# FeMTTU/femus

Hardware: AMD Instinct MI355X
Metric: assembled DOFs/sec + V-cycle SpMV GB/s (% HBM peak), 3D Poisson Q2 (higher is better)
Workload: dtype f64

## Files before the change

### femus_amd/csrc/fh_assemble.hip

```cpp
#include "fh_internal.h"
#include "fh_fe.h"
#include "fh_expr_device.h"
#include <algorithm>

struct SfTab { double L[3][4], D[3][4]; };

struct fh_assembler_s {
  fh_ctx_t ctx = nullptr;
  int geom = 0, fe = 0, order = 0, dim = 3, nc = 27, ng = 64, nloc = 27;
  int nel = 0, nnode = 0, ndof = 0;
  int ncolors = 0;
  std::vector<int> color_ptr;
  int* d_color_elems = nullptr;
  int* d_elem_dof = nullptr;
  double* d_coords = nullptr;
  double* d_w = nullptr;
  double* d_phi = nullptr;
  double* d_dphi = nullptr;
  int* d_emap = nullptr;
  int* d_iota = nullptr;
  int ncp = 28;
  int* d_adj_ptr = nullptr;
  int* d_adj_ei = nullptr;
  unsigned char* d_rowmap = nullptr;
// ... 9 lines not shown
  double *d_gal_val = nullptr, *d_gal_res = nullptr, *d_gal_dense = nullptr;
  int kstride = 27;
  double* d_Fbuf = nullptr;
  bool two_pass = false;
  bool fused = false;
  bool kbuf_valid = false;
  bool rows_used_since = false;
  int last_path = 0;
  int cl_ncl = 0, cl_nm = 0, cl_ns = 0, cl_nprow = 0;
  int cl_sup_shift = 0;
  int cl_walk_shift = 0;
  size_t cl_ncarried = 0;
  size_t cl_npart = 0;
  unsigned* d_cl_sinfo = nullptr;
  void *d_cl_dtab = nullptr, *d_cl_fblk = nullptr, *d_cl_oblk = nullptr;
  int *d_cl_vdst = nullptr, *d_cl_fdst = nullptr;
  unsigned long long* d_cl_vdst64 = nullptr;
  double* cl_val_base = nullptr;
  unsigned char *d_cl_map = nullptr, *d_cl_pmap = nullptr;
  unsigned char* d_cl_mapb = nullptr;
  unsigned short* d_cl_gtab = nullptr;
  bool cl_all_rows = false;
  bool macro_valid = false;
  fh_mat_t cl_mat_of_macro = nullptr;
  uint64_t macro_val_gen = 0;
  double* d_Pbuf = nullptr;
  int* d_cl_prow = nullptr;
  unsigned* d_cl_pstart = nullptr;
  int last_source_kind = 0;
  double last_params[2] = {1.0, 0.0};
// ... 1584 lines not shown
constexpr int CL_LV = CL_ZC + 2;
constexpr size_t CL_OFF_DT = (size_t)(CL_LV + CL_NBLK) * sizeof(double);
constexpr size_t CL_OFF_RB = CL_OFF_DT + (size_t)CL_NS_MAX * 8;
constexpr size_t CL_OFF_FB = CL_OFF_RB + (size_t)CL_NM_MAX * 8;
constexpr size_t CL_OFF_FL = CL_OFF_FB + (size_t)CL_NM_MAX * 4;
constexpr size_t CL_OFF_OV = CL_OFF_FL + (size_t)CL_NM_MAX * 16;
constexpr size_t cl_lds_bytes() { return CL_OFF_OV + (size_t)CL_NBLK * 16; }
static_assert((CL_LV + CL_NBLK) * 8 < (1 << 17), "cluster kernel: LDS byte addresses of the stagings and the long-sum cells fit 17 bits");
static_assert(CL_ZC < (1 << 16), "cluster kernel: 16-bit double indices of the address blocks");
static_assert(cl_lds_bytes() <= 160 * 1024, "cluster kernel: LDS budget");
static_assert((CL_TAB % 2) == 0 && (CL_UVS % 2) == 0, "cluster kernel: 16-byte alignment of the wave regions");

struct ClParams {
  int ncl, ns, nm;
  int sup_shift;
  const uint2* dtab;
  const uint4* fblk;
  const uint4* oblk;
  const unsigned* sinfo;
  const unsigned long long* vdst;
  const int* fdst;
  const uint4* map;
  const uint4* mapb;
  double* Pbuf;
  double* res;
  unsigned long long* stamps;
};

__device__ __forceinline__ double cl_sum8(const char* S, const uint4 a, double t) {
  const unsigned w[4] = {a.x, a.y, a.z, a.w};
// ... 225 lines not shown
        cl_gdouble* dst = (cl_gdouble*)vb[i];
        if (P.debug & 64) *dst = vv[i];
        else if (!(P.debug & 4)) __builtin_nontemporal_store(vv[i], dst);
        else if (vv[i] == 1.2345e300) *dst = vv[i];
      }
      if (CARRY && lane < 16) {
        cl_gdouble* dst = (cl_gdouble*)(fvv < 0 ? C.Pbuf + (size_t)(fvv & 0x7fffffff) : C.res + (size_t)(fvv & 0x3fffffff));
        *dst = (fvv >= 0 && (fvv & 0x40000000)) ? fold + fsum : fsum;
      }
      sf_stamp<INS>(st, 15);
    }
    sf_stamp<INS>(st, 10);
    __syncthreads();
    sf_stamp<INS>(st, 11);
    dof_n = dof_nn;
    ndone++;
  }
  if (INS && C.stamps && lane == 0) {
    unsigned long long* o = C.stamps + ((size_t)blockIdx.x * NW + wave) * 20;
#pragma unroll
    for (int k = 0; k < 16; k++) o[k] = st.acc[k];
    o[16] = (unsigned long long)ndone;
  }
}

constexpr int RP_Q = 7;
template <int NT>
__global__ __launch_bounds__(256) void k_rows_partial(int nprow, const int* __restrict__ prow, const unsigned* __restrict__ pstart, const unsigned char* __restrict__ pmap,
                                                      const double* __restrict__ Pbuf, const int* __restrict__ rowptr, double* __restrict__ val, double* __restrict__ res, int nt) {
  __shared__ double acc[8][2][128];
// ... 290 lines not shown
    FH_CHECK_HIP(hipMemcpyAsync(&perr, d_perr, sizeof(int), hipMemcpyDeviceToHost, ctx->stream));
    FH_CHECK_HIP(hipStreamSynchronize(ctx->stream));
    if (perr) return 0;
  }
  FH_TRACE("cluster plan: clusters verified");
  std::vector<unsigned short> roff(CL_NM_MAX + 1, 0);
  std::vector<unsigned char> tcol;
  int nsingle[CL_NM_MAX] = {};
  struct U2 { unsigned x, y; };
  struct U4 { unsigned short a[8]; };
  std::vector<U2> dtab;
  U4 zblk;
  for (int q = 0; q < 8; q++) zblk.a[q] = (unsigned short)CL_ZC;
  std::vector<U4> fblk(CL_NM_MAX, zblk), oblk;
  auto stag = [&](int e, int tr, int tc) { return (unsigned)(CL_TAB + e * SF_WAVE + SF_XT + tr * KS + tc); };
  auto pack = [&](const std::vector<unsigned>& ad, U2* out) -> bool {
    if (ad.empty() || ad.size() > 8) return false;
    out->x = ad[0] * 8;
    out->y = (ad.size() > 1 ? ad[1] : (unsigned)CL_ZC) * 8;
    if (ad.size() > 2) {
      if ((int)oblk.size() >= CL_NBLK) return false;
      U4 b = zblk;
      for (size_t q = 0; q < ad.size(); q++) b.a[q] = (unsigned short)ad[q];
      out->x = (unsigned)(CL_LV + (int)oblk.size()) * 8;
      out->y = (unsigned)CL_ZC * 8;
      oblk.push_back(b);
    }
    return true;
  };
  int tof_e[CL_NE][CL_NM_MAX];
  for (int e = 0; e < CL_NE; e++) {
    for (int k = 0; k < nm; k++) tof_e[e][k] = -1;
    for (int t = 0; t < 27; t++) tof_e[e][tm[e][t]] = t;
  }
  for (int r = 0; r < nm; r++) {
    bool has[CL_NM_MAX] = {};
    for (int e = 0; e < CL_NE; e++)
      if (tof_e[e][r] >= 0)
        for (int t = 0; t < 27; t++) has[tm[e][t]] = true;
    for (int pass = 0; pass < 2; pass++) {
      for (int k = 0; k < nm; k++)
        if (has[k]) {
          std::vector<unsigned> ad;
          for (int e = 0; e < CL_NE; e++)
            if (tof_e[e][r] >= 0 && tof_e[e][k] >= 0) ad.push_back(stag(e, tof_e[e][r], tof_e[e][k]));
          if ((ad.size() > 1) != (pass == 1)) continue;
          U2 d;
          if (!pack(ad, &d)) return 0;
          dtab.push_back(d);
          tcol.push_back((unsigned char)k);
        }
      if (pass == 0) nsingle[r] = (int)dtab.size() - roff[r];
    }
    roff[r + 1] = (unsigned short)dtab.size();
    if (roff[r + 1] - roff[r] > 127) return 0;
    int nf = 0;
    for (int e = 0; e < CL_NE; e++)
      if (tof_e[e][r] >= 0) fblk[r].a[nf++] = (unsigned short)stag(e, tof_e[e][r], 27);
  }
  for (int r = nm; r < CL_NM_MAX; r++) roff[r + 1] = roff[nm];
  const int ns = (int)dtab.size();
  if (ns > CL_NS_MAX || ns >= (1 << 13)) return 0;
  oblk.resize(CL_NBLK, zblk);
  std::vector<unsigned> sinfo((size_t)CL_SPT * CL_T, (unsigned)(CL_NM_MAX - 1));
  {
    int sidx = 0;
    for (int pass = 0; pass < 2; pass++)
      for (int r = 0; r < nm; r++) {
        const int p0 = pass ? nsingle[r] : 0, p1 = pass ? roff[r + 1] - roff[r] : nsingle[r];
        for (int pp = p0; pp < p1; pp++) sinfo[sidx++] = (unsigned)r | ((unsigned)pp << 7) | ((unsigned)roff[r] << 14);
      }
  }
  FH_TRACE("cluster plan: template");
  for (int r = 0; r <= CL_NM_MAX; r++) T.roff[r] = roff[r];
  unsigned char* d_complete = nullptr;
  unsigned *d_rowsz = nullptr, *d_rowbase = nullptr;
  FH_TRY(dalloc((void**)&d_complete, (size_t)m));
  FH_TRY(dalloc((void**)&d_rowsz, (size_t)m * sizeof(unsigned)));
// ... 41 lines not shown
  FH_CHECK_HIP(hipMalloc(&as->d_cl_vdst, (size_t)ncl * CL_NM_MAX * sizeof(int)));
  FH_CHECK_HIP(hipMalloc(&as->d_cl_fdst, (size_t)ncl * CL_NM_MAX * sizeof(int)));
  hipLaunchKernelGGL(k_cl_dst, dim3(gq), dim3(256), 0, ctx->stream, ncl, m, d_cdof, as->d_adj_ptr, as->d_adj_ei, A->d_rowptr, T, d_complete, d_rowbase, sink,
                     as->d_cl_vdst, as->d_cl_fdst);
  FH_CHECK_HIP(hipGetLastError());
  FH_CHECK_HIP(hipStreamSynchronize(ctx->stream));
  FH_TRACE("cluster plan: destinations");
  auto up = [&](void** d, const void* h, size_t bytes) -> int {
    FH_CHECK_HIP(hipMalloc(d, bytes ? bytes : 8));
    if (bytes) FH_CHECK_HIP(hipMemcpy(*d, h, bytes, hipMemcpyHostToDevice));
    return 0;
  };
  FH_TRY(up((void**)&as->d_cl_dtab, dtab.data(), dtab.size() * sizeof(U2)));
  FH_TRY(up((void**)&as->d_cl_fblk, fblk.data(), fblk.size() * sizeof(U4)));
  FH_TRY(up((void**)&as->d_cl_oblk, oblk.data(), oblk.size() * sizeof(U4)));
  {
    std::vector<unsigned short> gtab((size_t)CL_NE * 27 * 27, (unsigned short)0xffff);
    for (int e = 0; e < CL_NE; e++)
      for (int il = 0; il < 27; il++)
        for (int ic = 0; ic < 27; ic++) {
          const int r = tm[e][T.tof[il]], k = tm[e][T.tof[ic]];
          int owner = -1;
          for (int e2 = 0; e2 < CL_NE && owner < 0; e2++)
            if (tof_e[e2][r] >= 0 && tof_e[e2][k] >= 0) owner = e2;
          if (owner != e) continue;
          for (int idx = roff[r]; idx < roff[r + 1]; idx++)
            if (tcol[idx] == k) gtab[((size_t)e * 27 + il) * 27 + ic] = (unsigned short)idx;
        }
    FH_TRY(up((void**)&as->d_cl_gtab, gtab.data(), gtab.size() * sizeof(unsigned short)));
    as->cl_all_rows = (m == as->nnode);
// ... 25 lines not shown
    FH_CHECK_HIP(hipMemsetAsync(d_ncar, 0, sizeof(unsigned long long), ctx->stream));
    hipLaunchKernelGGL(k_cluster_maps, dim3(ncl), dim3(256), 0, ctx->stream, ncl, ns, nm, d_cdof, as->d_cl_sinfo, d_roff, d_tcol, as->d_cl_vdst, m, A->d_rowptr, A->d_col, d_complete,
                       as->d_adj_ptr, as->d_adj_ei, as->d_elem_dof, nloc, reinterpret_cast<uint4*>(as->d_cl_map), reinterpret_cast<uint4*>(as->d_cl_mapb), as->d_cl_pmap, d_first, d_err);
    if (sup_shift > 0 && m > 0)
      hipLaunchKernelGGL(k_cl_cover, dim3(fh_div_up(m, 256)), dim3(256), 0, ctx->stream, m, A->d_rowptr, d_complete, d_first, d_err, d_ncar);
    FH_CHECK_HIP(hipGetLastError());
    int err = 0;
    unsigned long long ncar = 0;
    FH_CHECK_HIP(hipMemcpyAsync(&err, d_err, sizeof(int), hipMemcpyDeviceToHost, ctx->stream));
    FH_CHECK_HIP(hipMemcpyAsync(&ncar, d_ncar, sizeof(ncar), hipMemcpyDeviceToHost, ctx->stream));
    FH_CHECK_HIP(hipStreamSynchronize(ctx->stream));
    as->cl_ncarried = (size_t)ncar;
    for (void* q : {(void*)d_tcol, (void*)d_roff, (void*)d_err}) hipFree(q);
    if (err && sup_shift > 0) {
      FH_TRACE("fh_assembler_create: carried rows do not cover their CSR rows -- cluster plan without them");
      for (void** q : {(void**)&as->d_cl_dtab, (void**)&as->d_cl_fblk, (void**)&as->d_cl_sinfo, (void**)&as->d_cl_oblk, (void**)&as->d_cl_gtab, (void**)&as->d_cl_vdst, (void**)&as->d_cl_vdst64,
                       (void**)&as->d_cl_fdst, (void**)&as->d_cl_map, (void**)&as->d_cl_mapb, (void**)&as->d_cl_pmap, (void**)&as->d_Pbuf, (void**)&as->d_cl_prow, (void**)&as->d_cl_pstart}) {
        if (*q) FH_CHECK_HIP(hipFree(*q));
        *q = nullptr;
      }
      return cluster_plan_build(as, A, elem_dof, aptr, false);
    }
    if (err) {
      FH_TRACE("fh_assembler_create: cluster maps could not be placed in the matrix pattern -- two-pass assembly kept");
      return 0;
    }
  }
  as->cl_ncl = ncl;
  as->cl_nm = nm;
  as->cl_ns = ns;
  as->cl_npart = npart;
  as->cl_nprow = (int)prow.size();
  as->cl_sup_shift = sup_shift;
  if (sup_shift > 0 || ctx->assemble_carry < 100) as->cl_walk_shift = sup_shift;
  as->fused = true;
  FH_TRACE("fh_assembler_create: cluster plan (%d clusters, %d macro nodes, %d entries; super-clusters of %d: %zu carried entries; %zu partial entries, %d rows in the second pass)", ncl,
           nm, ns, 1 << sup_shift, as->cl_ncarried, npart, as->cl_nprow);
  return 0;
}

template <bool CARRY>
static int launch_cluster_stamped(fh_assembler_t as, const AsmParams& P, const ClParams& C0, int grid) {
  constexpr size_t lds = cl_lds_bytes();
  static bool attr_set[64] = {};
  const int dev = as->ctx->device & 63;
  if (!attr_set[dev]) {
    FH_CHECK_HIP(hipFuncSetAttribute(reinterpret_cast<const void*>(&k_cluster_q2hex_sf<0, true, true, CARRY>), hipFuncAttributeMaxDynamicSharedMemorySize, (int)lds));
    attr_set[dev] = true;
  }
  ClParams C = C0;
  const size_t nst = (size_t)grid * CL_NE * 20;
  FH_CHECK_HIP(hipMalloc(&C.stamps, nst * sizeof(unsigned long long)));
  FH_CHECK_HIP(hipMemsetAsync(C.stamps, 0, nst * sizeof(unsigned long long), as->ctx->stream));
  hipLaunchKernelGGL((k_cluster_q2hex_sf<0, true, true, CARRY>), dim3(grid), dim3(CL_T), lds, as->ctx->stream, P, as->sf_tab, as->d_sfLc, as->d_sfLi, C);
  FH_CHECK_HIP(hipGetLastError());
  std::vector<unsigned long long> h(nst);
  FH_CHECK_HIP(hipMemcpyAsync(h.data(), C.stamps, nst * sizeof(unsigned long long), hipMemcpyDeviceToHost, as->ctx->stream));
  FH_CHECK_HIP(hipStreamSynchronize(as->ctx->stream));
  FH_CHECK_HIP(hipFree(C.stamps));
  static const int order[16] = {0, 1, 2, 3, 4, 5, 6, 7, 8, 9, 12, 14, 13, 15, 10, 11};
  static const char* name[16] = {"loop top (previous barrier exit -> stamp)", "phase A: U (gather x, first contraction, sync)", "phase A: V (second contraction, sync)",
                                 "phase A: J, cofactors, division, D_q", "stage 1 (15 MFMA, writes, sync)", "source 2nd contraction + stages 2-3 (4 x 16 reads + 66 FMA)",
                                 "source 3rd contraction, sync", "destination loads issued, staging writes (18), sync", "residual K_e u, next nodes, destinations",
                                 "workgroup barrier 1 (waiting for the slowest wave)", "(end of the output phase)", "workgroup barrier 2",
                                 "output: descriptors + destinations read, residual entries and long sums", "output: both operands read, added", "output: barrier behind the long sums", "output: stores issued"};
  for (int half = 0; half < 2; half++) {
    double sum[16] = {0}, ncl = 0, tot = 0;
    for (size_t w = 0; w < (size_t)grid * CL_NE; w++) {
      if ((int)((w % CL_NE) / (CL_NE / 2)) != half) continue;
      for (int k = 0; k < 16; k++) sum[k] += (double)h[w * 20 + k];
      ncl += (double)h[w * 20 + 16];
    }
    for (int k = 0; k < 16; k++) tot += sum[k];
    fprintf(stderr, "k_cluster_q2hex_sf<0> phase stamps, waves %d..%d (%s): %d workgroups, %.0f wave-clusters, %.0f shader-clock ticks per cluster and wave\n", half * 4, half * 4 + 3,
            half && !(P.debug & 256) ? "phase A one cluster ahead, i.e. rows 1-3 run behind row 8" : "phase A in place", grid, ncl, tot / std::max(ncl, 1.0));
    for (int kk = 0; kk < 16; kk++) {
      const int k = order[kk];
      fprintf(stderr, "  %2d %-62s %9.1f  %5.1f %%\n", k, name[k], sum[k] / std::max(ncl, 1.0), 100.0 * sum[k] / std::max(tot, 1.0));
    }
  }
  return 0;
}

template <int SRC, bool CARRY>
static int launch_cluster_one(fh_assembler_t as, const AsmParams& P, const ClParams& C) {
  constexpr size_t lds = cl_lds_bytes();
  static bool attr_set[64] = {};
  const int dev = as->ctx->device & 63;
  if (!attr_set[dev]) {
    FH_CHECK_HIP(hipFuncSetAttribute(reinterpret_cast<const void*>(&k_cluster_q2hex_sf<SRC, false, true, CARRY>), hipFuncAttributeMaxDynamicSharedMemorySize, (int)lds));
    attr_set[dev] = true;
  }
  const int grid = std::max(1, std::min(C.ncl >> (CARRY ? C.sup_shift : 0), as->ctx->num_cu * as->ctx->assemble_sf_grid));
  if (SRC == 0 && (as->ctx->asm_debug & 128)) return launch_cluster_stamped<CARRY>(as, P, C, grid);
  hipLaunchKernelGGL((k_cluster_q2hex_sf<SRC, false, true, CARRY>), dim3(grid), dim3(CL_T), lds, as->ctx->stream, P, as->sf_tab, as->d_sfLc, as->d_sfLi, C);
  FH_CHECK_HIP(hipGetLastError());
  return 0;
}

__global__ void k_cluster_vdst(size_t n, const int* __restrict__ vdst, double* Pbuf, double* val, unsigned long long* __restrict__ out) {
  const size_t k = (size_t)blockIdx.x * blockDim.x + threadIdx.x;
  if (k >= n) return;
  const int v = vdst[k];
  out[k] = reinterpret_cast<unsigned long long>(v < 0 ? Pbuf + (size_t)(v & 0x7fffffff) : val + (size_t)v);
}

static int launch_cluster(fh_assembler_t as, const AsmParams& P, fh_mat_t A, double* res) {
  if (as->cl_val_base != A->d_val) {
    const size_t n = (size_t)as->cl_ncl * CL_NM_MAX;
    hipLaunchKernelGGL(k_cluster_vdst, dim3((unsigned)((n + 255) / 256)), dim3(256), 0, as->ctx->stream, n, as->d_cl_vdst, as->d_Pbuf, A->d_val, as->d_cl_vdst64);
    FH_CHECK_HIP(hipGetLastError());
    as->cl_val_base = A->d_val;
  }
  ClParams C;
  C.ncl = as->cl_ncl; C.ns = as->cl_ns; C.nm = as->cl_nm;
  C.dtab = reinterpret_cast<const uint2*>(as->d_cl_dtab); C.fblk = reinterpret_cast<const uint4*>(as->d_cl_fblk); C.oblk = reinterpret_cast<const uint4*>(as->d_cl_oblk);
  C.sinfo = as->d_cl_sinfo;
  C.vdst = as->d_cl_vdst64; C.fdst = as->d_cl_fdst; C.map = reinterpret_cast<const uint4*>(as->d_cl_map); C.mapb = reinterpret_cast<const uint4*>(as->d_cl_mapb);
  C.Pbuf = as->d_Pbuf; C.res = res;
  C.stamps = nullptr;
  C.sup_shift = as->cl_walk_shift;
  if (as->cl_sup_shift > 0 || (as->ctx->assemble_carry >= 200 && as->d_cl_mapb)) {
    if (P.source_kind == 4) FH_TRY((launch_cluster_one<2, true>(as, P, C)));
    else if (P.source_kind != 0) FH_TRY((launch_cluster_one<1, true>(as, P, C)));
    else FH_TRY((launch_cluster_one<0, true>(as, P, C)));
  } else if (P.source_kind == 4) FH_TRY((launch_cluster_one<2, false>(as, P, C)));
  else if (P.source_kind != 0) FH_TRY((launch_cluster_one<1, false>(as, P, C)));
  else FH_TRY((launch_cluster_one<0, false>(as, P, C)));
  if (as->cl_nprow > 0 && !(as->ctx->asm_debug & (2 | 8))) {
    if (!(as->ctx->asm_debug & 32))
      hipLaunchKernelGGL(k_rows_partial<0>, dim3(fh_div_up(as->cl_nprow, 16)), dim3(256), 0, as->ctx->stream, as->cl_nprow, as->d_cl_prow, as->d_cl_pstart,
                         as->d_cl_pmap, as->d_Pbuf, A->d_rowptr, A->d_val, res, 0);
    else
      hipLaunchKernelGGL(k_rows_partial<1>, dim3(fh_div_up(as->cl_nprow, 16)), dim3(256), 0, as->ctx->stream, as->cl_nprow, as->d_cl_prow, as->d_cl_pstart,
                         as->d_cl_pmap, as->d_Pbuf, A->d_rowptr, A->d_val, res, 1);
    FH_CHECK_HIP(hipGetLastError());
  }
  return 0;
}

template <int SRC>
__global__ __launch_bounds__(256) void k_elem_q2hex_affine(AsmParams P, const double* __restrict__ Mab, const double* __restrict__ mphi) {
  constexpr int NC = 27, DIM = 3, EB = 16, NE = NC * NC;
// ... 614 lines not shown
extern "C" int fh_assembler_destroy(fh_assembler_t as) {
  if (!as) return 0;
  hipStreamSynchronize(as->ctx->stream);
  if (as->d_color_elems) hipFree(as->d_color_elems);
  hipFree(as->d_elem_dof);
  hipFree(as->d_coords);
  hipFree(as->d_w);
  hipFree(as->d_phi);
  hipFree(as->d_dphi);
  if (as->d_emap) hipFree(as->d_emap);
  for (void* q : {(void*)as->d_aff_elems, (void*)as->d_gen_elems, (void*)as->d_Mab, (void*)as->d_mphi, (void*)as->d_mfT, (void*)as->d_mfPhi, (void*)as->d_mfSFc, (void*)as->d_mfSFi, (void*)as->d_sfLc, (void*)as->d_sfLi})
    if (q) hipFree(q);
  if (as->d_prog) hipFree(as->d_prog);
  if (as->d_prog_consts) hipFree(as->d_prog_consts);
  hipFree(as->d_iota);
  for (void* q : {(void*)as->d_cl_dtab, (void*)as->d_cl_fblk, (void*)as->d_cl_sinfo, (void*)as->d_cl_oblk, (void*)as->d_cl_gtab, (void*)as->d_cl_vdst, (void*)as->d_cl_vdst64, (void*)as->d_cl_fdst, (void*)as->d_cl_map, (void*)as->d_cl_mapb, (void*)as->d_cl_pmap,
                  (void*)as->d_Pbuf, (void*)as->d_cl_prow, (void*)as->d_cl_pstart})
    if (q) hipFree(q);
  for (void* q : {(void*)as->d_adj_ptr, (void*)as->d_adj_ei, (void*)as->d_rowmap, (void*)as->d_Kbuf, (void*)as->d_Fbuf, (void*)as->d_slot, (void*)as->d_gal_child,
                  (void*)as->d_gal_cnt, (void*)as->d_gal_row, (void*)as->d_gal_fb, (void*)as->d_gal_cb, (void*)as->d_gal_val, (void*)as->d_gal_res, (void*)as->d_gal_dense,
                  (void*)as->d_gal_fmask})
    if (q) hipFree(q);
  delete as;
  return 0;
}

static int assemble_poisson_core(fh_assembler_t as, fh_vec_t sol, int source_kind, const double* params, fh_mat_t A, fh_vec_t res);

extern "C" int fh_assemble_poisson(fh_assembler_t as, fh_vec_t sol, int source_kind, const double* params, fh_mat_t A, fh_vec_t res) {
  FH_REQUIRE(source_kind >= 0 && source_kind <= 3, "fh_assemble_poisson: unknown source kind %d", source_kind);
// ... 1657 lines not shown
```

### femus_amd/csrc/fh_core.hip

```cpp
#include <cstdlib>
#include "fh_internal.h"
#include <chrono>
#include <cstdlib>
#include <cstdarg>
#include <cmath>

static thread_local char g_err[1024] = "";

void fh_set_error(const char* fmt, ...) {
  va_list ap;
  va_start(ap, fmt);
  vsnprintf(g_err, sizeof(g_err), fmt, ap);
  va_end(ap);
}

extern "C" const char* fh_last_error(void) { return g_err; }

bool fh_trace_on() {
  static const bool on = [] {
    const char* e = getenv("FEMUS_HIP_TRACE");
    return e && *e && *e != '0';
  }();
  return on;
}
// ... 181 lines not shown
  else if (!strcmp(name, "spmv_kernel")) c->spmv_kernel = (int)value;
  else if (!strcmp(name, "spmv_nt")) c->spmv_nt = (int)value;
  else if (!strcmp(name, "spmv_share")) c->spmv_share = (int)value;
  else if (!strcmp(name, "spmv_threads")) c->spmv_threads = (int)value;
  else if (!strcmp(name, "assemble_emap")) c->assemble_emap = (int)value;
  else if (!strcmp(name, "asm_debug")) c->asm_debug = (int)value;
  else if (!strcmp(name, "debug_poison")) c->debug_poison = (int)value;
  else if (!strcmp(name, "assemble_two_pass")) c->assemble_two_pass = (int)value;
  else if (!strcmp(name, "assemble_sym")) c->assemble_sym = (int)value;
  else if (!strcmp(name, "assemble_mfma")) c->assemble_mfma = (int)value;
  else if (!strcmp(name, "assemble_kpad")) c->assemble_kpad = (int)value;
  else if (!strcmp(name, "assemble_rows2")) c->assemble_rows2 = (int)value;
  else if (!strcmp(name, "assemble_sf")) c->assemble_sf = (int)value;
  else if (!strcmp(name, "assemble_rows_nt")) c->assemble_rows_nt = (int)value;
  else if (!strcmp(name, "assemble_fused")) c->assemble_fused = (int)value;
  else if (!strcmp(name, "assemble_sf_grid")) c->assemble_sf_grid = std::max(1, (int)value);
  else if (!strcmp(name, "assemble_sumfac")) c->assemble_sumfac = (int)value;
  else if (!strcmp(name, "galerkin_mfma")) c->galerkin_mfma = (int)value;
  else if (!strcmp(name, "gj_block")) c->gj_block = (int)value;
  else if (!strcmp(name, "vanka_persistent")) c->vanka_persistent = (int)value;
  else if (!strcmp(name, "coarse_reduce")) c->coarse_reduce = (int)value;
  else if (!strcmp(name, "coarse_nd")) c->coarse_nd = (int)value;
  else if (!strcmp(name, "coarse_nd_min")) c->coarse_nd_min = (int)value;
  else if (!strcmp(name, "coarse_direct")) c->coarse_direct = (int)value;
  else if (!strcmp(name, "gmres_device")) c->gmres_device = (int)value;
  else if (!strcmp(name, "galerkin_macro")) c->galerkin_macro = (int)value;
  else if (!strcmp(name, "vanka_fused")) c->vanka_fused = (int)value;
  else if (!strcmp(name, "coarse_direct_min")) c->coarse_direct_min = (int)value;
  else if (!strcmp(name, "coarse_nd_streams")) c->coarse_nd_streams = (int)value;
  else if (!strcmp(name, "patch_invert_lds")) c->patch_invert_lds = (int)value;
// ... 344 lines not shown
```

### femus_amd/csrc/fh_internal.h

```cpp
#pragma once
#include <hip/hip_runtime.h>
#include <cstdint>
#include <cstdio>
#include <cstdlib>
#include <cstring>
#include <new>
#include <stdexcept>
#include <string>
#include <algorithm>
#include <vector>
#include "../../include/femus_hip.h"

void fh_set_error(const char* fmt, ...);

#define FH_CHECK_HIP(expr)                                                                        \
  do {                                                                                            \
    hipError_t _e = (expr);                                                                       \
    if (_e != hipSuccess) {                                                                       \
      fh_set_error("%s:%d: %s failed: %s", __FILE__, __LINE__, #expr, hipGetErrorString(_e));     \
      return 1;                                                                                   \
    }                                                                                             \
  } while (0)

#define FH_REQUIRE(cond, ...)                                                                     \
// ... 50 lines not shown
  int spmv_share = 1;
  int spmv_nt = 0;
  int assemble_emap = 1;
  int asm_debug = 0;
  int debug_poison = 0;
  int assemble_mfma = 12;
  int assemble_rows_nt = 1;
  int assemble_sf_grid = 1;
  int assemble_sf = 8;
  int assemble_sumfac = 1;
  int assemble_rows2 = 1;
  int assemble_kpad = 1;
  int assemble_sym = 1;
  int assemble_two_pass = 1;
  int assemble_fused = 1;
  int ilu_ahead = 2;
  int tri_runs = 1;
  int assemble_carry = -1;
  int assemble_affine = 0;
  int gj_symmetric = 1;
  int galerkin_mfma = 1;
  int patch_invert_lds = 1;
  int coarse_nd = 8;
  int coarse_nd_streams = 0;
  int coarse_nd_min = 1024;
  int vanka_fused = 1;
  int galerkin_macro = 1;
  int gmres_device = 1;
  int coarse_direct = 1;
  int coarse_direct_min = 8192;
// ... 124 lines not shown
```

Baseline: 817.7 million.

## Add software-pipelined cluster assembly kernel with packed symmetric staging

```diff
diff --git a/femus_amd/csrc/fh_assemble.hip b/femus_amd/csrc/fh_assemble.hip
--- a/femus_amd/csrc/fh_assemble.hip
+++ b/femus_amd/csrc/fh_assemble.hip
@@ -47,6 +47,7 @@
   size_t cl_npart = 0;
   unsigned* d_cl_sinfo = nullptr;
   void *d_cl_dtab = nullptr, *d_cl_fblk = nullptr, *d_cl_oblk = nullptr;
+  void *d_cl_dtabp = nullptr, *d_cl_fblkp = nullptr, *d_cl_oblkp = nullptr;
   int *d_cl_vdst = nullptr, *d_cl_fdst = nullptr;
   unsigned long long* d_cl_vdst64 = nullptr;
   double* cl_val_base = nullptr;
@@ -1661,6 +1662,7 @@
 struct ClParams {
   int ncl, ns, nm;
   int sup_shift;
+  const unsigned* dtabp;
   const uint2* dtab;
   const uint4* fblk;
   const uint4* oblk;
@@ -1916,6 +1918,298 @@
     __syncthreads();
     sf_stamp<INS>(st, 11);
     dof_n = dof_nn;
+    ndone++;
+  }
+  if (INS && C.stamps && lane == 0) {
+    unsigned long long* o = C.stamps + ((size_t)blockIdx.x * NW + wave) * 20;
+#pragma unroll
+    for (int k = 0; k < 16; k++) o[k] = st.acc[k];
+    o[16] = (unsigned long long)ndone;
+  }
+}
+
+constexpr int CP_NT = 27 * 28 / 2;
+constexpr int CP_ES = CP_NT + 28;
+constexpr int CP_ST = 0;
+constexpr int CP_ZC = CP_ST + CL_NE * CP_ES;
+constexpr int CP_LV = CP_ZC + 2;
+constexpr int CP_TAB = CP_LV + CL_NBLK;
+constexpr int CP_W = CP_TAB + CL_TAB;
+constexpr size_t CP_OFF_DT = (size_t)(CP_W + CL_NE * SF_WAVE) * sizeof(double);
+constexpr size_t CP_OFF_RB = CP_OFF_DT + (size_t)CL_NS_MAX * 4;
+constexpr size_t CP_OFF_FB = CP_OFF_RB + (size_t)CL_NM_MAX * 8;
+constexpr size_t CP_OFF_FL = CP_OFF_FB + (size_t)CL_NM_MAX * 4;
+constexpr size_t CP_OFF_OV = CP_OFF_FL + (size_t)CL_NM_MAX * 16;
+constexpr size_t CP_OFF_SI = CP_OFF_OV + (size_t)CL_NBLK * 16;
+constexpr size_t cp_lds_bytes() { return CP_OFF_SI + (size_t)CL_SPT * CL_T * 4; }
+static_assert((CP_LV + CL_NBLK) * 8 <= 0xffff, "pipelined cluster kernel: 16-bit byte addresses of the stagings, the zero cell and the long-sum cells");
+static_assert(cp_lds_bytes() <= 160 * 1024, "pipelined cluster kernel: LDS budget");
+static_assert((CP_ES % 2) == 0 && (CP_TAB % 2) == 0 && (CP_W % 2) == 0, "pipelined cluster kernel: 16-byte alignment of the regions");
+__host__ __device__ constexpr int cp_packed(int r, int c) { return r >= c ? r * (r + 1) / 2 + c : c * (c + 1) / 2 + r; }
+
+template <int SRC, bool INS = false, bool CARRY = false>
+__global__ __launch_bounds__(CL_T) void k_cluster_q2hex_pipe(AsmParams P, SfTab tab, const double* __restrict__ lanec, const int* __restrict__ lanei, ClParams C) {
+  constexpr int NC = 27, DIM = 3, KS = MF_KS, NW = CL_NE;
+  constexpr bool REGC = true;
+  extern __shared__ __attribute__((aligned(16))) double sf_smem[];
+  double* SFl = sf_smem + CP_TAB;
+  int* SFi = reinterpret_cast<int*>(SFl + (SF_NLC - CL_LC0) * 64);
+  char* Sb = reinterpret_cast<char*>(sf_smem);
+  unsigned* dtab = reinterpret_cast<unsigned*>(Sb + CP_OFF_DT);
+  unsigned long long* rb = reinterpret_cast<unsigned long long*>(Sb + CP_OFF_RB);
+  int* fb = reinterpret_cast<int*>(Sb + CP_OFF_FB);
+  uint4* fblk = reinterpret_cast<uint4*>(Sb + CP_OFF_FL);
+  uint4* oblk = reinterpret_cast<uint4*>(Sb + CP_OFF_OV);
+  unsigned* sitab = reinterpret_cast<unsigned*>(Sb + CP_OFF_SI);
+  const int tid = threadIdx.x;
+  for (int k = tid; k < CL_SPT * CL_T; k += CL_T) sitab[k] = C.sinfo[k];
+  for (int k = tid; k < (SF_NLC - CL_LC0) * 64; k += CL_T) SFl[k] = lanec[CL_LC0 * 64 + k];
+  for (int k = tid; k < SF_NLI * 64; k += CL_T) SFi[k] = lanei[k];
+  for (int k = tid; k < C.ns; k += CL_T) dtab[k] = C.dtabp[k];
+  if (tid < CL_NM_MAX) fblk[tid] = C.fblk[tid];
+  if (tid < CL_NBLK) oblk[tid] = C.oblk[tid];
+  if (tid < 2) sf_smem[CP_ZC + tid] = 0.0;
+  __syncthreads();
+  const int lane = tid & 63;
+  const int wave = __builtin_amdgcn_readfirstlane(tid >> 6);
+  double* xt = sf_smem + CP_W + wave * SF_WAVE;
+  double* R = xt + SF_XT;
+  double* Ks = sf_smem + CP_ST + wave * CP_ES;
+  const double* LCl = SFl + lane - CL_LC0 * 64;
+  const int* LIl = SFi + lane;
+  double rcA[19], rcZ[8], rcY[16];
+#pragma unroll
+  for (int r = 0; r < 19; r++) rcA[r] = lanec[r * 64 + lane];
+#pragma unroll
+  for (int r = 0; r < 8; r++) rcZ[r] = lanec[(19 + r) * 64 + lane];
+#pragma unroll
+  for (int r = 0; r < 16; r++) rcY[r] = lanec[(27 + r) * 64 + lane];
+  unsigned pk0 = (unsigned)lanei[5 * 64 + lane] | ((unsigned)lanei[6 * 64 + lane] << 8) | ((unsigned)lanei[15 * 64 + lane] << 16) | ((unsigned)lanei[14 * 64 + lane] << 24) |
+                 ((lanei[9 * 64 + lane] != 0 ? 1u : 0u) << 29);
+  unsigned pk1;
+  {
+    const int based = lanei[7 * 64 + lane];
+    pk1 = (unsigned)(based / KS) | ((unsigned)(based % KS) << 8);
+  }
+  unsigned pk2 = (unsigned)lanei[lane] | ((unsigned)lanei[64 + lane] << 6) | ((unsigned)lanei[2 * 64 + lane] << 12) | ((unsigned)lanei[3 * 64 + lane] << 18) |
+                 ((unsigned)lanei[4 * 64 + lane] << 24);
+  const int nodeofl = (int)((pk0 >> 24) & 31u);
+  const int cstride = gridDim.x;
+  const int sh = CARRY ? C.sup_shift : 0;
+  const int nsup = C.ncl >> sh;
+  if ((int)blockIdx.x >= nsup) return;
+  const int nit = ((nsup - 1 - (int)blockIdx.x) / cstride + 1) << sh;
+  auto cl_at = [&](int it) {
+    it = min(it, nit - 1);
+    return ((((int)blockIdx.x + (it >> sh) * cstride)) << sh) + (it & ((1 << sh) - 1));
+  };
+  SfStamps st;
+  if (INS) {
+#pragma unroll
+    for (int k = 0; k < 16; k++) st.acc[k] = 0;
+    st.prev = __builtin_amdgcn_s_memtime();
+  }
+  auto element = [&](double (&Kb)[3][3], double& fsrc) {
+    CL_OPAQUE(pk0);
+    CL_OPAQUE(pk2);
+    const int esym = (int)(pk0 & 255u), ens = (int)((pk0 >> 8) & 255u), ensT = (int)((pk0 >> 16) & 255u);
+    const int eout = (lane >> 4) * SF_ES + (lane & 15);
+    double Dr[7];
+    sf_phase_a<SRC, REGC, INS>(P, LCl, CL_IDXA(), rcA, xt, R, Dr, &st);
+    wave_lds_sync();
+    sf_stages<SRC, REGC, INS>(P, tab, LCl, LIl, rcZ, rcY, esym, ens, ensT, eout, R, lane, Dr, Kb, fsrc, &st);
+    sf_stamp<INS>(st, 6);
+  };
+  auto stage_out = [&](const double (&Kb)[3][3], const double fsrc) {
+    CL_OPAQUE(pk0);
+    CL_OPAQUE(pk1);
+    const bool diag = ((pk0 >> 29) & 1u) != 0;
+    const int p = (int)(pk1 & 255u), p2 = (int)(pk1 >> 8);
+    const int bl = (p * (p + 1) >> 1) + p2, bu = (p2 * (p2 + 1) >> 1) + p;
+#pragma unroll
+    for (int a = 0; a < 3; a++)
+#pragma unroll
+      for (int a2 = 0; a2 < 3; a2++) {
+        const double v = (a2 < a && diag) ? Kb[a2][a] : Kb[a][a2];
+        const int idx = a > a2 ? bl + 9 * a * p + (9 * a) * (9 * a + 1) / 2 + 9 * a2 : bu + 9 * a2 * p2 + (9 * a2) * (9 * a2 + 1) / 2 + 9 * a;
+        Ks[idx] = v;
+      }
+    wave_lds_sync();
+    sf_stamp<INS>(st, 7);
+    const int t = min(lane & 31, NC - 1);
+    double ku = 0.0;
+    if (P.sol) {
+      const int h = lane >> 5;
+      const double* ur = xt + 84 + h * 14;
+      const int tt = (t * (t + 1)) >> 1;
+#pragma unroll
+      for (int g = 0; g < 14; g++) {
+        const bool live = g < 13 || h == 0;
+        const int c = h * 14 + g;
+        const int idx = c <= t ? tt + c : ((c * (c + 1)) >> 1) + t;
+        const double v = live ? Ks[idx] : 0.0, uu = live ? ur[g] : 0.0;
+        ku += v * uu;
+      }
+      ku += __shfl_xor(ku, 32, 64);
+    }
+    Ks[CP_NT + t] = -(ku + fsrc);
+  };
+  auto dst_load = [&](int c, unsigned long long& vd, int& fd) {
+    const int tm = tid & (CL_NM_MAX - 1);
+    vd = C.vdst[(size_t)c * CL_NM_MAX + tm];
+    fd = C.fdst[(size_t)c * CL_NM_MAX + tm];
+  };
+  int dof_n;
+  {
+    const int dof = P.elem_dof[(size_t)(cl_at(0) * NW + wave) * P.nloc + nodeofl];
+    if (lane < NC) {
+      xt[lane] = P.coords[(size_t)dof * DIM];
+      xt[28 + lane] = P.coords[(size_t)dof * DIM + 1];
+      xt[56 + lane] = P.coords[(size_t)dof * DIM + 2];
+      xt[84 + lane] = P.sol ? P.sol[dof] : 0.0;
+    }
+    dof_n = P.elem_dof[(size_t)(cl_at(1) * NW + wave) * P.nloc + nodeofl];
+  }
+  wave_lds_sync();
+  double Kb[3][3], fsrc;
+  {
+    unsigned long long vd;
+    int fd;
+    dst_load(cl_at(0), vd, fd);
+    const double nx0 = P.coords[(size_t)dof_n * DIM], nx1 = P.coords[(size_t)dof_n * DIM + 1], nx2 = P.coords[(size_t)dof_n * DIM + 2];
+    const double nu = P.sol ? P.sol[dof_n] : 0.0;
+    const int dof_nn = P.elem_dof[(size_t)(cl_at(2) * NW + wave) * P.nloc + nodeofl];
+    element(Kb, fsrc);
+    stage_out(Kb, fsrc);
+    if (lane < NC) {
+      xt[lane] = nx0;
+      xt[28 + lane] = nx1;
+      xt[56 + lane] = nx2;
+      xt[84 + lane] = nu;
+    }
+    if (tid < CL_NM_MAX) {
+      rb[tid] = vd;
+      fb[tid] = fd;
+    }
+    dof_n = dof_nn;
+  }
+  __syncthreads();
+  int ndone = 0;
+  typedef __attribute__((address_space(1))) double cl_gdouble;
+#pragma unroll 1
+  for (int it = 0; it < nit; it++) {
+    const int cl = cl_at(it);
+    const bool more = it + 1 < nit;
+    const uint4 mp_cur = C.map[(size_t)cl * CL_T + tid];
+    const uint4 mq_cur = CARRY ? C.mapb[(size_t)cl * CL_T + tid] : make_uint4(0u, 0u, 0u, 0u);
+    const int fv_own = CARRY ? C.fdst[(size_t)cl * CL_NM_MAX + wave * 16 + (lane & 15)] : 0;
+    sf_stamp<INS>(st, 0);
+    double nx0 = 0.0, nx1 = 0.0, nx2 = 0.0, nu = 0.0;
+    int dof_nn = 0;
+    if (more) {
+      nx0 = P.coords[(size_t)dof_n * DIM];
+      nx1 = P.coords[(size_t)dof_n * DIM + 1];
+      nx2 = P.coords[(size_t)dof_n * DIM + 2];
+      nu = P.sol ? P.sol[dof_n] : 0.0;
+      dof_nn = P.elem_dof[(size_t)(cl_at(it + 3) * NW + wave) * P.nloc + nodeofl];
+      element(Kb, fsrc);
+      if (lane < NC) {
+        xt[lane] = nx0;
+        xt[28 + lane] = nx1;
+        xt[56 + lane] = nx2;
+      }
+    }
+    unsigned long long vd_nx = 0;
+    int fd_nx = 0;
+    if (more) dst_load(cl_at(it + 1), vd_nx, fd_nx);
+    if (!(P.debug & 2)) {
+      const int frow = wave * 16 + (lane & 15);
+      const uint4 sumblk = (lane & 16) ? oblk[frow] : fblk[frow];
+      const unsigned mw[4] = {mp_cur.x, mp_cur.y, mp_cur.z, mp_cur.w};
+      const unsigned mq[4] = {mq_cur.x, mq_cur.y, mq_cur.z, mq_cur.w};
+      double fold = 0.0;
+      if (CARRY && lane < 16 && fv_own >= 0 && (fv_own & 0x40000000))
+        fold = __hip_atomic_load((const cl_gdouble*)(C.res + (size_t)(fv_own & 0x3fffffff)), __ATOMIC_RELAXED, __HIP_MEMORY_SCOPE_AGENT);
+      unsigned dd[CL_SPT];
+      unsigned long long vb[CL_SPT];
+      double accv[CARRY ? CL_SPT : 1];
+#pragma unroll
+      for (int i = 0; i < CL_SPT; i++) {
+        const unsigned si = sitab[i * CL_T + tid];
+        const int j = (mw[i >> 2] >> (8 * (i & 3))) & 255;
+        const int p = (si >> 7) & 127;
+        const int pos = CARRY ? (int)((mq[i >> 2] >> (8 * (i & 3))) & 255) : p;
+        dd[i] = dtab[(si >> 14) + j];
+        vb[i] = rb[si & 127] + (unsigned long long)(pos * 8);
+      }
+      if (CARRY) {
+#pragma unroll
+        for (int i = 0; i < CL_SPT; i++) {
+          accv[i] = 0.0;
+          if (((mw[2] >> (16 + i)) & 1u) && !(P.debug & 512)) accv[i] = __hip_atomic_load((const cl_gdouble*)vb[i], __ATOMIC_RELAXED, __HIP_MEMORY_SCOPE_AGENT);
+        }
+      }
+      double fsum;
+      int fvv;
+      {
+        const double v = cl_sum8(Sb, sumblk, 0.0);
+        const int fv = CARRY ? fv_own : fb[frow];
+        double* dst = fv < 0 ? C.Pbuf + (size_t)(fv & 0x7fffffff) : C.res + (size_t)(CARRY ? (fv & 0x3fffffff) : fv);
+        if (!CARRY) { if (lane < 16) *dst = v; }
+        if (lane >= 16 && lane < 32) sf_smem[CP_LV + frow] = v;
+        fsum = v;
+        fvv = fv;
+      }
+      if (INS) {
+        asm volatile("" ::"v"(dd[CL_SPT - 1]), "v"(vb[CL_SPT - 1]));
+        sf_stamp<INS>(st, 12);
+      }
+      __syncthreads();
+      sf_stamp<INS>(st, 14);
+      double vv[CL_SPT], ww[CL_SPT];
+#pragma unroll
+      for (int i = 0; i < CL_SPT; i++) {
+        vv[i] = *reinterpret_cast<const double*>(Sb + (dd[i] & 0xffffu));
+        ww[i] = *reinterpret_cast<const double*>(Sb + (dd[i] >> 16));
+      }
+#pragma unroll
+      for (int i = 0; i < CL_SPT; i++) vv[i] += ww[i];
+      if (CARRY) {
+#pragma unroll
+        for (int i = 0; i < CL_SPT; i++) vv[i] = accv[i] + vv[i];
+      }
+      if (INS) {
+        asm volatile("" ::"v"(vv[CL_SPT - 1]), "v"(vv[0]));
+        sf_stamp<INS>(st, 13);
+      }
+#pragma unroll
+      for (int i = 0; i < CL_SPT; i++) {
+        cl_gdouble* dst = (cl_gdouble*)vb[i];
+        if (P.debug & 64) *dst = vv[i];
+        else if (!(P.debug & 4)) __builtin_nontemporal_store(vv[i], dst);
+        else if (vv[i] == 1.2345e300) *dst = vv[i];
+      }
+      if (CARRY && lane < 16) {
+        cl_gdouble* dst = (cl_gdouble*)(fvv < 0 ? C.Pbuf + (size_t)(fvv & 0x7fffffff) : C.res + (size_t)(fvv & 0x3fffffff));
+        *dst = (fvv >= 0 && (fvv & 0x40000000)) ? fold + fsum : fsum;
+      }
+      sf_stamp<INS>(st, 15);
+    }
+    sf_stamp<INS>(st, 10);
+    __syncthreads();
+    sf_stamp<INS>(st, 9);
+    if (more) {
+      stage_out(Kb, fsrc);
+      if (lane < NC) xt[84 + lane] = nu;
+      if (tid < CL_NM_MAX) {
+        rb[tid] = vd_nx;
+        fb[tid] = fd_nx;
+      }
+      dof_n = dof_nn;
+    }
+    sf_stamp<INS>(st, 8);
+    __syncthreads();
+    sf_stamp<INS>(st, 11);
     ndone++;
   }
   if (INS && C.stamps && lane == 0) {
@@ -2236,6 +2530,20 @@
   for (int q = 0; q < 8; q++) zblk.a[q] = (unsigned short)CL_ZC;
   std::vector<U4> fblk(CL_NM_MAX, zblk), oblk;
   auto stag = [&](int e, int tr, int tc) { return (unsigned)(CL_TAB + e * SF_WAVE + SF_XT + tr * KS + tc); };
+  std::vector<unsigned> dtabp;
+  U4 zblkp;
+  for (int q = 0; q < 8; q++) zblkp.a[q] = (unsigned short)CP_ZC;
+  std::vector<U4> fblkp(CL_NM_MAX, zblkp), oblkp;
+  auto stagp = [&](int e, int tr, int tc) { return (unsigned)(CP_ST + e * CP_ES + (tc == 27 ? CP_NT + tr : cp_packed(tr, tc))); };
+  auto packp = [&](const std::vector<unsigned>& ad, unsigned* out) {
+    *out = (ad[0] * 8) | ((ad.size() > 1 ? ad[1] : (unsigned)CP_ZC) * 8) << 16;
+    if (ad.size() > 2) {
+      U4 b = zblkp;
+      for (size_t q = 0; q < ad.size(); q++) b.a[q] = (unsigned short)ad[q];
+      *out = ((unsigned)(CP_LV + (int)oblkp.size()) * 8) | ((unsigned)CP_ZC * 8) << 16;
+      oblkp.push_back(b);
+    }
+  };
   auto pack = [&](const std::vector<unsigned>& ad, U2* out) -> bool {
     if (ad.empty() || ad.size() > 8) return false;
     out->x = ad[0] * 8;
@@ -2263,13 +2571,19 @@
     for (int pass = 0; pass < 2; pass++) {
       for (int k = 0; k < nm; k++)
         if (has[k]) {
-          std::vector<unsigned> ad;
+          std::vector<unsigned> ad, adp;
           for (int e = 0; e < CL_NE; e++)
-            if (tof_e[e][r] >= 0 && tof_e[e][k] >= 0) ad.push_back(stag(e, tof_e[e][r], tof_e[e][k]));
+            if (tof_e[e][r] >= 0 && tof_e[e][k] >= 0) {
+              ad.push_back(stag(e, tof_e[e][r], tof_e[e][k]));
+              adp.push_back(stagp(e, tof_e[e][r], tof_e[e][k]));
+            }
           if ((ad.size() > 1) != (pass == 1)) continue;
           U2 d;
           if (!pack(ad, &d)) return 0;
           dtab.push_back(d);
+          unsigned dp;
+          packp(adp, &dp);
+          dtabp.push_back(dp);
           tcol.push_back((unsigned char)k);
         }
       if (pass == 0) nsingle[r] = (int)dtab.size() - roff[r];
@@ -2278,12 +2592,16 @@
     if (roff[r + 1] - roff[r] > 127) return 0;
     int nf = 0;
     for (int e = 0; e < CL_NE; e++)
-      if (tof_e[e][r] >= 0) fblk[r].a[nf++] = (unsigned short)stag(e, tof_e[e][r], 27);
+      if (tof_e[e][r] >= 0) {
+        fblkp[r].a[nf] = (unsigned short)stagp(e, tof_e[e][r], 27);
+        fblk[r].a[nf++] = (unsigned short)stag(e, tof_e[e][r], 27);
+      }
   }
   for (int r = nm; r < CL_NM_MAX; r++) roff[r + 1] = roff[nm];
   const int ns = (int)dtab.size();
   if (ns > CL_NS_MAX || ns >= (1 << 13)) return 0;
   oblk.resize(CL_NBLK, zblk);
+  oblkp.resize(CL_NBLK, zblkp);
   std::vector<unsigned> sinfo((size_t)CL_SPT * CL_T, (unsigned)(CL_NM_MAX - 1));
   {
     int sidx = 0;
@@ -2355,6 +2673,9 @@
   FH_TRY(up((void**)&as->d_cl_dtab, dtab.data(), dtab.size() * sizeof(U2)));
   FH_TRY(up((void**)&as->d_cl_fblk, fblk.data(), fblk.size() * sizeof(U4)));
   FH_TRY(up((void**)&as->d_cl_oblk, oblk.data(), oblk.size() * sizeof(U4)));
+  FH_TRY(up((void**)&as->d_cl_dtabp, dtabp.data(), dtabp.size() * sizeof(unsigned)));
+  FH_TRY(up((void**)&as->d_cl_fblkp, fblkp.data(), fblkp.size() * sizeof(U4)));
+  FH_TRY(up((void**)&as->d_cl_oblkp, oblkp.data(), oblkp.size() * sizeof(U4)));
   {
     std::vector<unsigned short> gtab((size_t)CL_NE * 27 * 27, (unsigned short)0xffff);
     for (int e = 0; e < CL_NE; e++)
@@ -2410,7 +2731,7 @@
     for (void* q : {(void*)d_tcol, (void*)d_roff, (void*)d_err}) hipFree(q);
     if (err && sup_shift > 0) {
       FH_TRACE("fh_assembler_create: carried rows do not cover their CSR rows -- cluster plan without them");
-      for (void** q : {(void**)&as->d_cl_dtab, (void**)&as->d_cl_fblk, (void**)&as->d_cl_sinfo, (void**)&as->d_cl_oblk, (void**)&as->d_cl_gtab, (void**)&as->d_cl_vdst, (void**)&as->d_cl_vdst64,
+      for (void** q : {(void**)&as->d_cl_dtab, (void**)&as->d_cl_fblk, (void**)&as->d_cl_dtabp, (void**)&as->d_cl_fblkp, (void**)&as->d_cl_oblkp, (void**)&as->d_cl_sinfo, (void**)&as->d_cl_oblk, (void**)&as->d_cl_gtab, (void**)&as->d_cl_vdst, (void**)&as->d_cl_vdst64,
                        (void**)&as->d_cl_fdst, (void**)&as->d_cl_map, (void**)&as->d_cl_mapb, (void**)&as->d_cl_pmap, (void**)&as->d_Pbuf, (void**)&as->d_cl_prow, (void**)&as->d_cl_pstart}) {
         if (*q) FH_CHECK_HIP(hipFree(*q));
         *q = nullptr;
@@ -2435,31 +2756,44 @@
   return 0;
 }
 
-template <bool CARRY>
+template <bool PIPE, bool CARRY>
+static const void* cluster_kernel() {
+  return PIPE ? reinterpret_cast<const void*>(&k_cluster_q2hex_pipe<0, true, CARRY>) : reinterpret_cast<const void*>(&k_cluster_q2hex_sf<0, true, true, CARRY>);
+}
+template <bool PIPE, bool CARRY>
 static int launch_cluster_stamped(fh_assembler_t as, const AsmParams& P, const ClParams& C0, int grid) {
-  constexpr size_t lds = cl_lds_bytes();
+  constexpr size_t lds = PIPE ? cp_lds_bytes() : cl_lds_bytes();
   static bool attr_set[64] = {};
   const int dev = as->ctx->device & 63;
   if (!attr_set[dev]) {
-    FH_CHECK_HIP(hipFuncSetAttribute(reinterpret_cast<const void*>(&k_cluster_q2hex_sf<0, true, true, CARRY>), hipFuncAttributeMaxDynamicSharedMemorySize, (int)lds));
+    FH_CHECK_HIP(hipFuncSetAttribute(cluster_kernel<PIPE, CARRY>(), hipFuncAttributeMaxDynamicSharedMemorySize, (int)lds));
     attr_set[dev] = true;
   }
   ClParams C = C0;
   const size_t nst = (size_t)grid * CL_NE * 20;
   FH_CHECK_HIP(hipMalloc(&C.stamps, nst * sizeof(unsigned long long)));
   FH_CHECK_HIP(hipMemsetAsync(C.stamps, 0, nst * sizeof(unsigned long long), as->ctx->stream));
-  hipLaunchKernelGGL((k_cluster_q2hex_sf<0, true, true, CARRY>), dim3(grid), dim3(CL_T), lds, as->ctx->stream, P, as->sf_tab, as->d_sfLc, as->d_sfLi, C);
+  if (PIPE) hipLaunchKernelGGL((k_cluster_q2hex_pipe<0, true, CARRY>), dim3(grid), dim3(CL_T), lds, as->ctx->stream, P, as->sf_tab, as->d_sfLc, as->d_sfLi, C);
+  else hipLaunchKernelGGL((k_cluster_q2hex_sf<0, true, true, CARRY>), dim3(grid), dim3(CL_T), lds, as->ctx->stream, P, as->sf_tab, as->d_sfLc, as->d_sfLi, C);
   FH_CHECK_HIP(hipGetLastError());
   std::vector<unsigned long long> h(nst);
   FH_CHECK_HIP(hipMemcpyAsync(h.data(), C.stamps, nst * sizeof(unsigned long long), hipMemcpyDeviceToHost, as->ctx->stream));
   FH_CHECK_HIP(hipStreamSynchronize(as->ctx->stream));
   FH_CHECK_HIP(hipFree(C.stamps));
-  static const int order[16] = {0, 1, 2, 3, 4, 5, 6, 7, 8, 9, 12, 14, 13, 15, 10, 11};
-  static const char* name[16] = {"loop top (previous barrier exit -> stamp)", "phase A: U (gather x, first contraction, sync)", "phase A: V (second contraction, sync)",
-                                 "phase A: J, cofactors, division, D_q", "stage 1 (15 MFMA, writes, sync)", "source 2nd contraction + stages 2-3 (4 x 16 reads + 66 FMA)",
-                                 "source 3rd contraction, sync", "destination loads issued, staging writes (18), sync", "residual K_e u, next nodes, destinations",
-                                 "workgroup barrier 1 (waiting for the slowest wave)", "(end of the output phase)", "workgroup barrier 2",
-                                 "output: descriptors + destinations read, residual entries and long sums", "output: both operands read, added", "output: barrier behind the long sums", "output: stores issued"};
+  static const int order_sf[16] = {0, 1, 2, 3, 4, 5, 6, 7, 8, 9, 12, 14, 13, 15, 10, 11};
+  static const char* name_sf[16] = {"loop top (previous barrier exit -> stamp)", "phase A: U (gather x, first contraction, sync)", "phase A: V (second contraction, sync)",
+                                    "phase A: J, cofactors, division, D_q", "stage 1 (15 MFMA, writes, sync)", "source 2nd contraction + stages 2-3 (4 x 16 reads + 66 FMA)",
+                                    "source 3rd contraction, sync", "destination loads issued, staging writes (18), sync", "residual K_e u, next nodes, destinations",
+                                    "workgroup barrier 1 (waiting for the slowest wave)", "(end of the output phase)", "workgroup barrier 2",
+                                    "output: descriptors + destinations read, residual entries and long sums", "output: both operands read, added", "output: barrier behind the long sums", "output: stores issued"};
+  static const int order_pipe[16] = {0, 1, 2, 3, 4, 5, 6, 12, 14, 13, 15, 10, 9, 7, 8, 11};
+  static const char* name_pipe[16] = {"loop top (barrier exit, map / slot loads issued)", "phase A: U (gather x, first contraction, sync)", "phase A: V (second contraction, sync)",
+                                      "phase A: J, cofactors, division, D_q", "stage 1 (15 MFMA, writes, sync)", "source 2nd contraction + stages 2-3 (4 x 16 reads + 66 FMA)",
+                                      "source 3rd contraction, sync", "packed staging writes (9), sync", "residual K_e u, next nodes, destinations",
+                                      "workgroup barrier 1 (behind the output)", "(end of the output phase)", "workgroup barrier 2 (behind the stagings)",
+                                      "output: descriptors + destinations read, residual entries and long sums", "output: both operands read, added", "output: barrier behind the long sums", "output: stores issued"};
+  const int* order = PIPE ? order_pipe : order_sf;
+  const char* const* name = PIPE ? name_pipe : name_sf;
   for (int half = 0; half < 2; half++) {
     double sum[16] = {0}, ncl = 0, tot = 0;
     for (size_t w = 0; w < (size_t)grid * CL_NE; w++) {
@@ -2468,8 +2802,9 @@
       ncl += (double)h[w * 20 + 16];
     }
     for (int k = 0; k < 16; k++) tot += sum[k];
-    fprintf(stderr, "k_cluster_q2hex_sf<0> phase stamps, waves %d..%d (%s): %d workgroups, %.0f wave-clusters, %.0f shader-clock ticks per cluster and wave\n", half * 4, half * 4 + 3,
-            half && !(P.debug & 256) ? "phase A one cluster ahead, i.e. rows 1-3 run behind row 8" : "phase A in place", grid, ncl, tot / std::max(ncl, 1.0));
+    fprintf(stderr, "%s<0> phase stamps, waves %d..%d (%s): %d workgroups, %.0f wave-clusters, %.0f shader-clock ticks per cluster and wave\n",
+            PIPE ? "k_cluster_q2hex_pipe" : "k_cluster_q2hex_sf", half * 4, half * 4 + 3,
+            PIPE ? "pipelined" : half && !(P.debug & 256) ? "phase A one cluster ahead, i.e. rows 1-3 run behind row 8" : "phase A in place", grid, ncl, tot / std::max(ncl, 1.0));
     for (int kk = 0; kk < 16; kk++) {
       const int k = order[kk];
       fprintf(stderr, "  %2d %-62s %9.1f  %5.1f %%\n", k, name[k], sum[k] / std::max(ncl, 1.0), 100.0 * sum[k] / std::max(tot, 1.0));
@@ -2478,20 +2813,34 @@
   return 0;
 }
 
-template <int SRC, bool CARRY>
+template <int SRC, bool PIPE, bool CARRY>
 static int launch_cluster_one(fh_assembler_t as, const AsmParams& P, const ClParams& C) {
-  constexpr size_t lds = cl_lds_bytes();
+  constexpr size_t lds = PIPE ? cp_lds_bytes() : cl_lds_bytes();
   static bool attr_set[64] = {};
   const int dev = as->ctx->device & 63;
   if (!attr_set[dev]) {
-    FH_CHECK_HIP(hipFuncSetAttribute(reinterpret_cast<const void*>(&k_cluster_q2hex_sf<SRC, false, true, CARRY>), hipFuncAttributeMaxDynamicSharedMemorySize, (int)lds));
+    const void* k = PIPE ? reinterpret_cast<const void*>(&k_cluster_q2hex_pipe<SRC, false, CARRY>) : reinterpret_cast<const void*>(&k_cluster_q2hex_sf<SRC, false, true, CARRY>);
+    FH_CHECK_HIP(hipFuncSetAttribute(k, hipFuncAttributeMaxDynamicSharedMemorySize, (int)lds));
     attr_set[dev] = true;
   }
   const int grid = std::max(1, std::min(C.ncl >> (CARRY ? C.sup_shift : 0), as->ctx->num_cu * as->ctx->assemble_sf_grid));
-  if (SRC == 0 && (as->ctx->asm_debug & 128)) return launch_cluster_stamped<CARRY>(as, P, C, grid);
-  hipLaunchKernelGGL((k_cluster_q2hex_sf<SRC, false, true, CARRY>), dim3(grid), dim3(CL_T), lds, as->ctx->stream, P, as->sf_tab, as->d_sfLc, as->d_sfLi, C);
+  if (SRC == 0 && (as->ctx->asm_debug & 128)) return launch_cluster_stamped<PIPE, CARRY>(as, P, C, grid);
+  if (PIPE) hipLaunchKernelGGL((k_cluster_q2hex_pipe<SRC, false, CARRY>), dim3(grid), dim3(CL_T), lds, as->ctx->stream, P, as->sf_tab, as->d_sfLc, as->d_sfLi, C);
+  else hipLaunchKernelGGL((k_cluster_q2hex_sf<SRC, false, true, CARRY>), dim3(grid), dim3(CL_T), lds, as->ctx->stream, P, as->sf_tab, as->d_sfLc, as->d_sfLi, C);
   FH_CHECK_HIP(hipGetLastError());
   return 0;
+}
+
+template <bool PIPE>
+static int launch_cluster_src(fh_assembler_t as, const AsmParams& P, const ClParams& C, bool carry) {
+  if (carry) {
+    if (P.source_kind == 4) return launch_cluster_one<2, PIPE, true>(as, P, C);
+    if (P.source_kind != 0) return launch_cluster_one<1, PIPE, true>(as, P, C);
+    return launch_cluster_one<0, PIPE, true>(as, P, C);
+  }
+  if (P.source_kind == 4) return launch_cluster_one<2, PIPE, false>(as, P, C);
+  if (P.source_kind != 0) return launch_cluster_one<1, PIPE, false>(as, P, C);
+  return launch_cluster_one<0, PIPE, false>(as, P, C);
 }
 
 __global__ void k_cluster_vdst(size_t n, const int* __restrict__ vdst, double* Pbuf, double* val, unsigned long long* __restrict__ out) {
@@ -2510,19 +2859,19 @@
   }
   ClParams C;
   C.ncl = as->cl_ncl; C.ns = as->cl_ns; C.nm = as->cl_nm;
-  C.dtab = reinterpret_cast<const uint2*>(as->d_cl_dtab); C.fblk = reinterpret_cast<const uint4*>(as->d_cl_fblk); C.oblk = reinterpret_cast<const uint4*>(as->d_cl_oblk);
+  const bool pipe = as->ctx->cluster_pipeline != 0;
+  C.dtab = reinterpret_cast<const uint2*>(as->d_cl_dtab);
+  C.dtabp = reinterpret_cast<const unsigned*>(as->d_cl_dtabp);
+  C.fblk = reinterpret_cast<const uint4*>(pipe ? as->d_cl_fblkp : as->d_cl_fblk);
+  C.oblk = reinterpret_cast<const uint4*>(pipe ? as->d_cl_oblkp : as->d_cl_oblk);
   C.sinfo = as->d_cl_sinfo;
   C.vdst = as->d_cl_vdst64; C.fdst = as->d_cl_fdst; C.map = reinterpret_cast<const uint4*>(as->d_cl_map); C.mapb = reinterpret_cast<const uint4*>(as->d_cl_mapb);
   C.Pbuf = as->d_Pbuf; C.res = res;
   C.stamps = nullptr;
   C.sup_shift = as->cl_walk_shift;
-  if (as->cl_sup_shift > 0 || (as->ctx->assemble_carry >= 200 && as->d_cl_mapb)) {
-    if (P.source_kind == 4) FH_TRY((launch_cluster_one<2, true>(as, P, C)));
-    else if (P.source_kind != 0) FH_TRY((launch_cluster_one<1, true>(as, P, C)));
-    else FH_TRY((launch_cluster_one<0, true>(as, P, C)));
-  } else if (P.source_kind == 4) FH_TRY((launch_cluster_one<2, false>(as, P, C)));
-  else if (P.source_kind != 0) FH_TRY((launch_cluster_one<1, false>(as, P, C)));
-  else FH_TRY((launch_cluster_one<0, false>(as, P, C)));
+  const bool carry = as->cl_sup_shift > 0 || (as->ctx->assemble_carry >= 200 && as->d_cl_mapb);
+  if (pipe) FH_TRY(launch_cluster_src<true>(as, P, C, carry));
+  else FH_TRY(launch_cluster_src<false>(as, P, C, carry));
   if (as->cl_nprow > 0 && !(as->ctx->asm_debug & (2 | 8))) {
     if (!(as->ctx->asm_debug & 32))
       hipLaunchKernelGGL(k_rows_partial<0>, dim3(fh_div_up(as->cl_nprow, 16)), dim3(256), 0, as->ctx->stream, as->cl_nprow, as->d_cl_prow, as->d_cl_pstart,
@@ -3167,6 +3516,7 @@
   if (as->d_prog) hipFree(as->d_prog);
   if (as->d_prog_consts) hipFree(as->d_prog_consts);
   hipFree(as->d_iota);
+  for (void* q : {(void*)as->d_cl_dtabp, (void*)as->d_cl_fblkp, (void*)as->d_cl_oblkp}) if (q) hipFree(q);
   for (void* q : {(void*)as->d_cl_dtab, (void*)as->d_cl_fblk, (void*)as->d_cl_sinfo, (void*)as->d_cl_oblk, (void*)as->d_cl_gtab, (void*)as->d_cl_vdst, (void*)as->d_cl_vdst64, (void*)as->d_cl_fdst, (void*)as->d_cl_map, (void*)as->d_cl_mapb, (void*)as->d_cl_pmap,
                   (void*)as->d_Pbuf, (void*)as->d_cl_prow, (void*)as->d_cl_pstart})
     if (q) hipFree(q);
diff --git a/femus_amd/csrc/fh_core.hip b/femus_amd/csrc/fh_core.hip
--- a/femus_amd/csrc/fh_core.hip
+++ b/femus_amd/csrc/fh_core.hip
@@ -219,6 +219,7 @@
   else if (!strcmp(name, "assemble_sf")) c->assemble_sf = (int)value;
   else if (!strcmp(name, "assemble_rows_nt")) c->assemble_rows_nt = (int)value;
   else if (!strcmp(name, "assemble_fused")) c->assemble_fused = (int)value;
+  else if (!strcmp(name, "cluster_pipeline")) c->cluster_pipeline = (int)value;
   else if (!strcmp(name, "assemble_sf_grid")) c->assemble_sf_grid = std::max(1, (int)value);
   else if (!strcmp(name, "assemble_sumfac")) c->assemble_sumfac = (int)value;
   else if (!strcmp(name, "galerkin_mfma")) c->galerkin_mfma = (int)value;
diff --git a/femus_amd/csrc/fh_internal.h b/femus_amd/csrc/fh_internal.h
--- a/femus_amd/csrc/fh_internal.h
+++ b/femus_amd/csrc/fh_internal.h
@@ -88,6 +88,7 @@
   int assemble_sym = 1;
   int assemble_two_pass = 1;
   int assemble_fused = 1;
+  int cluster_pipeline = 1;
   int ilu_ahead = 2;
   int tri_runs = 1;
   int assemble_carry = -1;
```

New measurement: 817.6 million, median of 5. Within noise of the previous version (-0.0%).
